# q8888620002/Group-Attribution-for-Diffusion-Models

Measured on AMD Instinct MI355X. Metric: shapley_coalitions_per_hour, higher is better.
Workload: dtype f32; 1 GPU; CIFAR-20 DDPM sFT coalition (BASELINE configs[1]): gd_steps=1000 @B=128 + 10240 samples x 100 DDIM steps @B=32 (32 batches fused/launch), UNet2DModel widths [128, 256, 256, 256] 35.75M params fp32; step = 1/1000 coalition = 1 train step + 1 sampler step @B=1024, enqueued on 3 HIP streams (the train step belongs to a later coalition: independent work); coalitions_in_flight=3

## Files before the change

### group-attribution-for-diffusion-models_amd/csrc/norm.hip

```cpp
#include "gad_reduce.h"
#include "gemm_dev.h"

namespace {

constexpr int NT = 256;
constexpr int MAXC = 3072;

struct Geo {
  int B, HW, C, G, cpg, C4, tpr, rows_par, nch, ppc;
};

static Geo make_geo(const gad_groupnorm_args* a) {
  Geo g;
  g.B = a->B; g.HW = a->HW; g.C = a->C; g.G = a->G;
  g.cpg = a->C / a->G;
  g.C4 = a->C / 4;
  g.tpr = g.C4 < NT ? g.C4 : NT;
  g.rows_par = NT / g.tpr;
  int nch = 2048 / (a->B > 0 ? a->B : 1);
  int maxch = a->HW / (8 * g.rows_par > 32 ? 8 * g.rows_par : 32);
  if (nch > maxch) nch = maxch;
  if (nch < 1) nch = 1;
  g.ppc = (a->HW + nch - 1) / nch;
  g.nch = (a->HW + g.ppc - 1) / g.ppc;
  return g;
}

__device__ __forceinline__ const float* gn_src(const float* x, const float* x2, int C1, int C, int HW, int b, int c0, int* stride) {
  if (x2 == nullptr || c0 < C1) {
    const int w = x2 ? C1 : C;
    *stride = w;
    return x + ((long)b * HW) * w + c0;
  }
  *stride = C - C1;
  return x2 + ((long)b * HW) * (C - C1) + (c0 - C1);
}

__device__ __forceinline__ bool gn_far_mean(const f32x4& mu, const f32x4& rs) {
  const f32x4 t = (mu * rs) * (mu * rs);
  return !(fmaxf(fmaxf(t[0], t[1]), fmaxf(t[2], t[3])) <= GN_COND - 1.f);
}
__global__ __launch_bounds__(NT) void gn_stats_kernel(const float* __restrict__ x, float* __restrict__ part, Geo g,
                                                      const float* __restrict__ x2, int C1) {
  __shared__ float red[2 * MAXC];
  __shared__ float s_mean[256];
  __shared__ int s_ill;
  if (threadIdx.x == 0) s_ill = 0;
  int b = blockIdx.x / g.nch, ch = blockIdx.x - b * g.nch;
  int p0 = ch * g.ppc, p1 = min(g.HW, p0 + g.ppc);
  int tid = threadIdx.x;
  int prow = tid / g.tpr, cfirst = tid - prow * g.tpr;
  if (prow < g.rows_par) {
// ... 399 lines not shown
  __syncthreads();
  f32x4* img4 = reinterpret_cast<f32x4*>(gn_img);
  if (act) {
    const float r1 = s_rstd[q / s.qpg], m2 = s_mean[q / s.qpg];
    const f32x4 rs = f32x4{r1, r1, r1, r1}, mu2 = f32x4{m2, m2, m2, m2};
    const f32x4 ga = *reinterpret_cast<const f32x4*>(gamma + c0), be = *reinterpret_cast<const f32x4*>(beta + c0);
    const f32x4 scale = ga * rs, shift = be - scale * mu2;
    const bool far = gn_far_mean(mu2, rs);
#pragma unroll
    for (int i = 0; i < NV; ++i) {
      int p = pl + i * s.PL;
      if (p < s.HW) {
        f32x4 z = far ? (v[i] - mu2) * scale + be : v[i] * scale + shift;
        if (silu) {
#pragma unroll
          for (int e = 0; e < 4; ++e) z[e] = silu_f(z[e]);
        }
        const int yy = p / w.W, xx = p - yy * w.W;
        img4[(yy * w.W + (xx ^ ((xx >> 2) & 1))) * s.qpr + q] = z;
      }
    }
  }
  __syncthreads();
  const int H = s.HW / w.W;
  const int items = w.TH * w.TW * s.qpr;
  for (int it = tid; it < items; it += NTH) {
    const int tile = it / s.qpr, qq = it - tile * s.qpr;
    const int ty = tile / w.TW, tx = tile - ty * w.TW;
    f32x4 t[6][6];
#pragma unroll
    for (int dx = 0; dx < 6; ++dx) {
      const int xx = 4 * tx - 1 + dx;
      const bool xok = xx >= 0 && xx < w.W;
      const int xs = xx ^ ((xx >> 2) & 1);
      f32x4 d[6], col[6];
#pragma unroll
      for (int dy = 0; dy < 6; ++dy) {
        const int yy = 4 * ty - 1 + dy;
        const bool ok = xok && yy >= 0 && yy < H;
        d[dy] = ok ? img4[(yy * w.W + xs) * s.qpr + qq] : f32x4{0.f, 0.f, 0.f, 0.f};
      }
      gadk::wino4_bt(d, col);
#pragma unroll
      for (int i = 0; i < 6; ++i) t[i][dx] = col[i];
    }
    float* out = w.V + ((long)b * (w.TH * w.TW) + tile) * s.C + sl * s.SC + qq * 4;
#pragma unroll
    for (int i = 0; i < 6; ++i) {
      f32x4 vv[6];
      gadk::wino4_bt(t[i], vv);
#pragma unroll
      for (int j = 0; j < 6; ++j) *reinterpret_cast<f32x4*>(out + (long)(6 * i + j) * w.pos_stride) = vv[j];
    }
  }
}

static int make_slab_wino(const gad_groupnorm_args* a, SlabGeo* out) {
  const int cpg = a->C / a->G, nth = 512;
  if (cpg % 4 != 0) return 0;
  int best_nv = 0;
  long best_score = -1;
  for (int k = 1; k * cpg <= a->C && k <= 64; ++k) {
    const int SC = k * cpg;
    if (a->C % SC != 0 || SC % 32 != 0) continue;
    if ((long)a->HW * SC * 4 > 128 * 1024) break;
    const int qpr = SC / 4;
    if (qpr > nth) break;
    const int PL = nth / qpr, nv = (a->HW + PL - 1) / PL;
    if (nv > 16) continue;
    const long blocks = (long)a->B * (a->C / SC);
    const long score = (blocks >= 512 ? (1L << 40) : blocks << 16) + SC;
    if (score > best_score) {
      best_score = score;
      best_nv = nv;
      int P2 = 1;
      while (P2 < PL) P2 <<= 1;
      *out = SlabGeo{a->HW, a->C, a->G, cpg, SC, qpr, PL, P2, a->C / SC, k, cpg / 4, 0};
    }
  }
  return !best_nv ? 0 : best_nv <= 4 ? 4 : best_nv <= 8 ? 8 : 16;
}

__device__ __forceinline__ float act_grad(float dy, float z, int silu) {
  if (!silu) return dy;
  float s = 1.f / (1.f + expf(-z));
  return dy * s * (1.f + z * (1.f - s));
}

template <int NV, int NTH>
__global__ __launch_bounds__(NTH) void gn_bwd_slab_kernel(const float* __restrict__ x, const float* __restrict__ dy,
                                                          float* __restrict__ dx, const float* __restrict__ gamma,
                                                          const float* __restrict__ beta, const float* __restrict__ mean,
                                                          const float* __restrict__ rstd, float* __restrict__ part,
                                                          SlabGeo s, int silu, const float* __restrict__ dx_add) {
  __shared__ f32x4 red_a[NTH], red_b[NTH];
  __shared__ float s_m1[64], s_m2[64];
  int b, sl;
  slab_of_block(s, b, sl);
  const int tid = threadIdx.x;
  const int pl = tid / s.qpr, q = tid - pl * s.qpr;
  const bool act = pl < s.PL;
  const int c0 = sl * s.SC + (act ? q : 0) * 4;
  const long base = ((long)b * s.HW) * s.C + c0;
  int gi[4];
  f32x4 mu, rs;
#pragma unroll
// ... 237 lines not shown
  dim3 grid(a->B * g.nch), block(NT);
  hipLaunchKernelGGL(gn_stats_kernel, grid, block, 0, st, a->x, (float*)a->ws, g, a->x2, a->C1);
  GAD_LAUNCH_CHECK("gn_stats");
  hipLaunchKernelGGL(gn_apply_kernel, grid, block, 0, st, a->x, a->y, a->gamma, a->beta, (const float*)a->ws, a->mean, a->rstd, g, a->eps, a->silu,
                     a->x2, a->C1);
  GAD_LAUNCH_CHECK("gn_apply");
  return 0;
}


static bool gn_wino_shapes_ok(const gad_groupnorm_args* a, int32_t W) {
  if (!a || a->B <= 0 || a->HW <= 0 || a->C <= 0 || a->G <= 0 || a->C % a->G != 0 || a->C % 32 != 0 || a->G > 256) return false;
  if (W <= 0 || a->HW % W != 0 || (W & 3) || ((a->HW / W) & 3)) return false;
  if (a->x2 && !(a->C1 > 0 && a->C1 < a->C && a->C1 % 4 == 0 && (a->C - a->C1) % 4 == 0)) return false;
  return true;
}
extern "C" int gad_groupnorm_wino4_ok(const gad_groupnorm_args* a, int32_t W) {
  SlabGeo sg;
  return gn_wino_shapes_ok(a, W) && make_slab_wino(a, &sg) ? 1 : 0;
}
extern "C" int gad_groupnorm_silu_wino4(const gad_groupnorm_args* a, float* V, int32_t W, void* stream) {
  GAD_CHECK(a && a->x && a->gamma && a->beta && a->mean && a->rstd && V, "gad_groupnorm_silu_wino4: null pointer");
  GAD_CHECK(gn_wino_shapes_ok(a, W), "gad_groupnorm_silu_wino4: shapes outside the plan (C %% 32, W and H multiples of 4; C=%d G=%d HW=%d W=%d)", a->C, a->G, a->HW, W);
  GAD_CHECK(gad_aligned16(a->x) && gad_aligned16(V) && gad_aligned16(a->gamma) && gad_aligned16(a->beta) && (!a->x2 || gad_aligned16(a->x2)),
            "gad_groupnorm_silu_wino4: pointers must be 16-byte aligned");
  SlabGeo sg;
  const int nv = make_slab_wino(a, &sg);
  GAD_CHECK(nv, "gad_groupnorm_silu_wino4: no slab plan (gad_groupnorm_wino4_ok tells)");
  GnWino w;
  w.V = V; w.W = W; w.TH = (a->HW / W) / 4; w.TW = W / 4;
  w.pos_stride = (long)a->B * w.TH * w.TW * a->C;
  const int c1 = a->x2 ? a->C1 : a->C;
  const int bytes = a->HW * sg.SC * (int)sizeof(float);
  hipStream_t st = (hipStream_t)stream;
  dim3 grid(a->B * sg.nslab), block(512);
#define GAD_GNW(NV_)                                                                                                        \
  do {                                                                                                                      \
    static int lds_set = 0;                                                                                                 \
    if (bytes > lds_set) {                                                                                                  \
      hipError_t e = hipFuncSetAttribute(reinterpret_cast<const void*>(gn_wino4_kernel<NV_>), hipFuncAttributeMaxDynamicSharedMemorySize, bytes); \
      GAD_CHECK(e == hipSuccess, "gad_groupnorm_silu_wino4: cannot reserve %d bytes of LDS: %s", bytes, hipGetErrorString(e)); \
      lds_set = bytes;                                                                                                      \
    }                                                                                                                       \
    hipLaunchKernelGGL((gn_wino4_kernel<NV_>), grid, block, bytes, st, a->x, a->x2, c1, a->gamma, a->beta, a->mean, a->rstd, sg, a->eps, a->silu, w); \
  } while (0)
  if (nv == 4) GAD_GNW(4);
  else if (nv == 8) GAD_GNW(8);
  else GAD_GNW(16);
#undef GAD_GNW
  GAD_LAUNCH_CHECK("gn_wino4");
  return 0;
}

extern "C" int gad_groupnorm_silu_bwd(const gad_groupnorm_args* a, void* stream) {
  if (check(a, "gad_groupnorm_silu_bwd")) return 1;
  GAD_CHECK(a->dy && gad_aligned16(a->dy) && ((a->dgamma == nullptr) == (a->dbeta == nullptr)), "gad_groupnorm_silu_bwd: null/unaligned grad pointer");
  GAD_CHECK(!a->dx_add || gad_aligned16(a->dx_add), "gad_groupnorm_silu_bwd: dx_add must be 16-byte aligned");
  Geo g = make_geo(a);
  hipStream_t st = (hipStream_t)stream;
  if (!(a->flags & GAD_GN_TWO_PASS)) {
    SlabGeo sg;
    int nth = NT, nv = make_slab(a, &sg, NT, 16);
    if (!nv) { nth = 512; nv = make_slab(a, &sg, 512, 16); }
    if (nv) {
      float* part = (float*)a->ws;
      dim3 sgrid(a->B * sg.nslab);
#define GAD_GNB(NV_, NTH_) hipLaunchKernelGGL((gn_bwd_slab_kernel<NV_, NTH_>), sgrid, dim3(NTH_), 0, st, a->x, a->dy, a->y, a->gamma, \
                                              a->beta, a->mean, a->rstd, part, sg, a->silu, a->dx_add)
      if (nth == NT) {
        if (nv <= 4) GAD_GNB(4, NT);
        else GAD_GNB(16, NT);
      } else {
        GAD_GNB(16, 512);
      }
#undef GAD_GNB
      GAD_LAUNCH_CHECK("gn_bwd_slab");
      if (a->dgamma) {
        float* ws2 = part + (long)a->B * a->C * 2;
        gad_reduce::launch(part, a->dbeta, a->dgamma, 1, (long)a->B, 2 * a->C, ws2, st);
        GAD_LAUNCH_CHECK("gn_bwd_param");
      }
      return 0;
    }
  }
  dim3 grid(a->B * g.nch), block(NT);
  hipLaunchKernelGGL(gn_bwd_stats_kernel, grid, block, 0, st, a->x, a->dy, a->gamma, a->beta, a->mean, a->rstd, (float*)a->ws, g, a->silu);
  GAD_LAUNCH_CHECK("gn_bwd_stats");
  hipLaunchKernelGGL(gn_bwd_apply_kernel, grid, block, 0, st, a->x, a->dy, a->y, a->gamma, a->beta, a->mean, a->rstd, (const float*)a->ws, g, a->silu, a->dx_add);
  GAD_LAUNCH_CHECK("gn_bwd_apply");
  if (a->dgamma) {
    float* ws2 = (float*)a->ws + (long)a->B * g.nch * a->C * 2;
    gad_reduce::launch((const float*)a->ws, a->dbeta, a->dgamma, 1, (long)a->B * g.nch, 2 * a->C, ws2, st);
    GAD_LAUNCH_CHECK("gn_bwd_param");
  }
  return 0;
}
```

### group-attribution-for-diffusion-models_amd/gad/_capi.py

```python
import ctypes as C
import os

_HERE = os.path.dirname(os.path.abspath(__file__))
LIB_PATH = os.path.join(_HERE, "libgad_hip.so")


class GadError(RuntimeError):
    pass


class ConvGeom(C.Structure):
    _fields_ = [("H", C.c_int32), ("W", C.c_int32), ("C", C.c_int32), ("ldx", C.c_int32),
                ("Ho", C.c_int32), ("Wo", C.c_int32), ("KH", C.c_int32), ("KW", C.c_int32),
                ("stride", C.c_int32), ("pad_t", C.c_int32), ("pad_l", C.c_int32), ("upsample", C.c_int32)]


class GemmArgs(C.Structure):
    _fields_ = [("A", C.c_void_p), ("B", C.c_void_p), ("C", C.c_void_p),
                ("a_mode", C.c_int32), ("b_mode", C.c_int32),
                ("M", C.c_int32), ("N", C.c_int32), ("K", C.c_int32),
                ("lda", C.c_int32), ("ldb", C.c_int32), ("ldc", C.c_int32),
                ("batch", C.c_int32), ("batch_inner", C.c_int32),
                ("strideA0", C.c_int64), ("strideA1", C.c_int64), ("strideB0", C.c_int64),
                ("strideB1", C.c_int64), ("strideC0", C.c_int64), ("strideC1", C.c_int64),
# ... 58 lines not shown

class JLArgs(C.Structure):
    _fields_ = [("A", C.c_void_p), ("lda", C.c_int64), ("G", C.c_int32), ("P", C.c_int64), ("p0", C.c_int64),
                ("d", C.c_int32), ("seed", C.c_uint32), ("model_id", C.c_uint32), ("type", C.c_int32),
                ("accumulate", C.c_int32), ("out", C.c_void_p), ("workspace", C.c_void_p), ("workspace_bytes", C.c_int64)]


class HGemmSegArgs(C.Structure):
    _fields_ = [("A", C.c_void_p), ("B", C.c_void_p), ("C", C.c_void_p), ("ws", C.c_void_p), ("ws_bytes", C.c_int64),
                ("c_seg_stride", C.c_int64), ("M", C.c_int32), ("N", C.c_int32), ("L", C.c_int32), ("S", C.c_int32),
                ("lda", C.c_int32), ("ldb", C.c_int32), ("ldc", C.c_int32), ("alpha", C.c_float), ("accumulate", C.c_int32),
                ("splitk_hint", C.c_int32)]


class LoraDropoutArgs(C.Structure):
    _fields_ = [("x", C.c_void_p), ("ldx", C.c_int64), ("M", C.c_int64), ("C", C.c_int32), ("r", C.c_int32),
                ("n_proj", C.c_int32), ("layer", C.c_uint32), ("A", C.c_void_p * 4), ("mid", C.c_void_p * 4),
                ("dmid", C.c_void_p * 4), ("dA", C.c_void_p * 4), ("dx", C.c_void_p), ("ld_dx", C.c_int64), ("p", C.c_double),
                ("scale", C.c_float), ("seed", C.c_uint32), ("offset", C.c_uint32), ("max_blocks", C.c_int32),
                ("workspace", C.c_void_p), ("workspace_bytes", C.c_int64)]


JL_NORMAL, JL_RADEMACHER = 0, 1
POOL_MAX, POOL_AVG, POOL_AVG_VALID = 0, 1, 2
GELU_ERF, GELU_QUICK = 0, 1
SIM_X_F32, SIM_X_U8 = 0, 1

GEMM_NO_PATCH, GEMM_TAP_MAJOR_K, GEMM_SCALAR_EPILOGUE, GEMM_GENERAL_LOADERS, GN_TWO_PASS = 1, 2, 4, 8, 1
GEMM_NO_WINO = 16
GEMM_WINO_WGRAD = 32
GEMM_WINO_ONLY_INPUT, GEMM_WINO_SKIP_INPUT = 64, 128
A_KC, A_MC, A_CONV, A_CONVT = 0, 1, 2, 3
B_KC, B_MC, B_WDGRAD, B_CONV = 0, 1, 2, 3

_vp, _i32, _i64, _f32, _f64 = C.c_void_p, C.c_int32, C.c_int64, C.c_float, C.c_double

SIGNATURES = {
    "gad_version": (C.c_int, []),
    "gad_last_error": (C.c_char_p, []),
    "gad_gemm_workspace_bytes": (_i64, [C.POINTER(GemmArgs)]),
    "gad_gemm": (C.c_int, [C.POINTER(GemmArgs), _vp]),
    "gad_gemm_uses_bf16": (C.c_int, [C.POINTER(GemmArgs)]),
    "gad_gemm_kernel_id": (C.c_int, [C.POINTER(GemmArgs)]),
    "gad_gemm_wino_bytes": (_i64, [C.POINTER(GemmArgs)]),
    "gad_wino_weights": (C.c_int, [_vp, _vp, _vp, _i64, _vp]),
    "gad_wino4_weights": (C.c_int, [_vp, _vp, _vp, _i64, _vp]),
    "gad_groupnorm_one_pass": (C.c_int, [C.POINTER(GroupNormArgs)]),
    "gad_gemm_plan": (C.c_int, [C.POINTER(GemmArgs), C.POINTER(_i32), C.POINTER(_i32), C.POINTER(_i32)]),
    "gad_groupnorm_workspace_bytes": (_i64, [C.POINTER(GroupNormArgs)]),
    "gad_groupnorm_silu_fwd": (C.c_int, [C.POINTER(GroupNormArgs), _vp]),
    "gad_groupnorm_silu_bwd": (C.c_int, [C.POINTER(GroupNormArgs), _vp]),
    "gad_groupnorm_wino4_ok": (C.c_int, [C.POINTER(GroupNormArgs), C.c_int32]),
    "gad_groupnorm_silu_wino4": (C.c_int, [C.POINTER(GroupNormArgs), _vp, C.c_int32, _vp]),
    "gad_attention_supported": (C.c_int, [_i32]),
    "gad_attention_uses_bf16": (C.c_int, [C.POINTER(AttentionArgs), _i32]),
    "gad_attention_bwd_workspace_bytes": (_i64, [C.POINTER(AttentionArgs)]),
    "gad_attention_fwd": (C.c_int, [C.POINTER(AttentionArgs), _vp]),
    "gad_attention_bwd": (C.c_int, [C.POINTER(AttentionArgs), _vp]),
    "gad_attention_d512_supported": (C.c_int, [_i32]),
    "gad_attention_fwd_d512": (C.c_int, [C.POINTER(AttentionArgs), _vp]),
    "gad_attention_causal_supported": (C.c_int, [_i32, _i32]),
    "gad_attention_causal_fwd": (C.c_int, [C.POINTER(AttentionArgs), _vp]),
    "gad_softmax_fwd": (C.c_int, [_vp, _vp, _i64, _i32, _f32, _vp]),
    "gad_softmax_bwd": (C.c_int, [_vp, _vp, _vp, _i64, _i32, _f32, _vp]),
    "gad_layernorm_workspace_bytes": (_i64, [_i64, _i32]),
    "gad_layernorm_fwd": (C.c_int, [_vp, _vp, _vp, _vp, _vp, _vp, _i64, _i32, _f32, _vp]),
    "gad_layernorm_bwd": (C.c_int, [_vp, _vp, _vp, _vp, _vp, _vp, _vp, _vp, _i64, _i32, _vp, _i64, _vp]),
    "gad_geglu_fwd": (C.c_int, [_vp, _vp, _i64, _i32, _vp]),
    "gad_geglu_bwd": (C.c_int, [_vp, _vp, _vp, _i64, _i32, _vp]),
    "gad_timestep_embedding": (C.c_int, [_vp, _vp, _i32, _i32, _i32, _f32, _f32, _vp]),
    "gad_rotate_conv3x3": (C.c_int, [_vp, _vp, _vp, _i32, _vp]),
    "gad_silu_fwd": (C.c_int, [_vp, _vp, _i64, _vp]),
    "gad_silu_bwd": (C.c_int, [_vp, _vp, _vp, _i64, _vp]),
    "gad_concat_channels": (C.c_int, [_vp, _vp, _vp, _i64, _i32, _i32, _vp]),
    "gad_split_channels": (C.c_int, [_vp, _vp, _vp, _i64, _i32, _i32, _vp]),
    "gad_nchw_to_nhwc": (C.c_int, [_vp, _vp, _i32, _i32, _i32, _vp]),
    "gad_nhwc_to_nchw": (C.c_int, [_vp, _vp, _i32, _i32, _i32, _vp]),
    "gad_upsample2x_bwd": (C.c_int, [_vp, _vp, _i32, _i32, _i32, _i32, _vp]),
    "gad_colsum": (C.c_int, [_vp, _vp, _i32, _i64, _i32, _vp, _i64, _vp]),
    "gad_add_noise": (C.c_int, [_vp, _vp, _vp, _vp, _vp, _i32, _i64, _vp]),
    "gad_ddim_step": (C.c_int, [_vp, _vp, _vp, _i64, _f32, _f32, _f32, _vp]),
    "gad_cfg_ddim_step": (C.c_int, [_vp, _vp, _vp, _i64, _f32, _f32, _f32, _f32, _vp]),
    "gad_to_image01": (C.c_int, [_vp, _vp, _i64, _vp]),
    "gad_mse_fwd_bwd": (C.c_int, [_vp, _vp, _vp, _vp, _i64, _f32, _vp, _i64, _vp]),
    "gad_sumsq": (C.c_int, [_vp, _vp, _i64, _vp, _i64, _vp]),
    "gad_clip_adam_ema": (C.c_int, [C.POINTER(AdamArgs), _vp]),
    "gad_ema_update": (C.c_int, [_vp, _vp, _i64, _f32, _vp]),
    "gad_hgemm_workspace_bytes": (_i64, [C.POINTER(HGemmArgs)]),
    "gad_hgemm_plan": (C.c_int, [C.POINTER(HGemmArgs), C.POINTER(_i32), C.POINTER(_i32)]),
    "gad_hgemm": (C.c_int, [C.POINTER(HGemmArgs), _vp]),
    "gad_hgemm_tn_workspace_bytes": (_i64, [C.POINTER(HGemmArgs)]),
    "gad_hgemm_tn": (C.c_int, [C.POINTER(HGemmArgs), _vp]),
    "gad_hgemm_tn_seg_workspace_bytes": (_i64, [C.POINTER(HGemmSegArgs)]),
    "gad_hgemm_tn_seg": (C.c_int, [C.POINTER(HGemmSegArgs), _vp]),
    "gad_h_transpose": (C.c_int, [_vp, _vp, _i32, _i32, _i32, _i32, _i32, _vp]),
    "gad_h_cast": (C.c_int, [_vp, _vp, _i64, _i32, _vp]),
    "gad_h_shadow_pairs": (C.c_int, [_vp, _vp, _vp, _vp, _i32, _vp]),
    "gad_h_add": (C.c_int, [_vp, _vp, _vp, _i64, _vp]),
    "gad_h_groupnorm_workspace_bytes": (_i64, [C.POINTER(GroupNormArgs)]),
    "gad_h_groupnorm_silu_fwd": (C.c_int, [C.POINTER(GroupNormArgs), _vp]),
    "gad_h_groupnorm_silu_bwd": (C.c_int, [C.POINTER(GroupNormArgs), _vp]),
    "gad_h_layernorm_fwd": (C.c_int, [_vp, _vp, _vp, _vp, _vp, _vp, _i64, _i32, _f32, _vp]),
    "gad_h_layernorm_bwd": (C.c_int, [_vp, _vp, _vp, _vp, _vp, _vp, _vp, _i64, _i32, _vp]),
    "gad_h_geglu_fwd": (C.c_int, [_vp, _vp, _i64, _i32, _vp]),
    "gad_h_geglu_bwd": (C.c_int, [_vp, _vp, _vp, _i64, _i32, _vp]),
    "gad_h_upsample2x_bwd": (C.c_int, [_vp, _vp, _i32, _i32, _i32, _i32, _vp]),
# ... 58 lines not shown
```

### group-attribution-for-diffusion-models_amd/gad/ops.py

```python
from __future__ import annotations

import ctypes as C
import math
from typing import Optional

import torch

from . import _capi
from ._capi import (A_CONV, A_CONVT, A_KC, A_MC, B_CONV, B_KC, B_MC, B_WDGRAD, AdamArgs, ConvGeom, GemmArgs,
                    GroupNormArgs, check)
from .shadows import (WEIGHT_EPOCH, Shadow, cached, in_flat_buffer as _in_flat_buffer, weight_key, written,
                      written_everywhere)

_WS = {}
WS_BYTES = 1 << 30


def _stream():
    return C.c_void_p(torch.cuda.current_stream().cuda_stream)


_raw_stream = getattr(torch._C, "_cuda_getCurrentRawStream", None)


# ... 49 lines not shown

def _sink(param):
    if _PER_SAMPLE[0] is not None and param is not None and param.requires_grad:
        raise _capi.GadError("per-sample gradient sink: only the LoRA matrices of the half-precision activation path have "
                             "per-sample gradients (csrc/half.hip: gad_hgemm_tn_seg)")
    v = getattr(param, "_gad_sink", None) if (param is not None and _SINK_ACTIVE[0]) else None
    if v is None:
        return None, True
    first = getattr(param, "_gad_sink_epoch", -1) != _SINK_EPOCH[0]
    param._gad_sink_epoch = _SINK_EPOCH[0]
    return v, first


def _deliver(param, grad):
    v, first = _sink(param)
    if v is None:
        return grad
    if first:
        v.copy_(grad)
    else:
        v.add_(grad)
    return None


OPERAND_PRECISION = [0]


class operand_precision:

    def __init__(self, name):
        if name not in ("f32", "fp32", "no", "bf16", "bf16-operands", "bf16-activations"):
            raise ValueError(f"operand precision {name!r}: use 'f32', 'bf16' (= 'bf16-activations') or 'bf16-operands'")
        self.value = {"bf16": 2, "bf16-activations": 2, "bf16-operands": 1}.get(name, 0)

    def __enter__(self):
        self.prev = OPERAND_PRECISION[0]
        OPERAND_PRECISION[0] = self.value
        return self

    def __exit__(self, *exc):
        OPERAND_PRECISION[0] = self.prev
        return False


def set_operand_precision(name):
    OPERAND_PRECISION[0] = 0 if name in (None, "no", "f32", "fp32") else operand_precision("bf16" if name in ("fp16", "bf16") else name).value


def half_activations() -> bool:
    return OPERAND_PRECISION[0] == 2


KERNEL_FLAGS = {"gemm": 0, "gn": 0, "native_dgrad": False, "two_kernel_attn_bwd": False, "narrow_attn_fwd": False, "no_wino4": False,
                "no_gn_wino": False}


class kernel_flags:

    def __init__(self, no_patch=False, tap_major_k=False, gn_two_pass=False, scalar_epilogue=False, general_loaders=False,
                 native_dgrad=False, two_kernel_attn_bwd=False, narrow_attn_fwd=False, no_wino=False, no_wino4=False, no_gn_wino=False):
        gemm = ((_capi.GEMM_NO_PATCH if no_patch else 0) | (_capi.GEMM_TAP_MAJOR_K if tap_major_k else 0)
                | (_capi.GEMM_NO_WINO if no_wino else 0)
                | (_capi.GEMM_SCALAR_EPILOGUE if scalar_epilogue else 0)
                | (_capi.GEMM_GENERAL_LOADERS if general_loaders else 0))
        self.values = {"gemm": gemm, "gn": _capi.GN_TWO_PASS if gn_two_pass else 0, "native_dgrad": native_dgrad,
                       "two_kernel_attn_bwd": two_kernel_attn_bwd, "narrow_attn_fwd": narrow_attn_fwd, "no_wino4": no_wino4,
                       "no_gn_wino": no_gn_wino}

    def __enter__(self):
        self.prev = dict(KERNEL_FLAGS)
        KERNEL_FLAGS.update(self.values)
        return self

    def __exit__(self, *exc):
        KERNEL_FLAGS.update(self.prev)
        return False


SCRATCH_ALLOC = None
OUT_ALLOC = None
OUT_ALLOC_DT = None


ROUTE_STATS = None


def _scratch(kind, nbytes, device):
    if SCRATCH_ALLOC is not None:
        return SCRATCH_ALLOC(kind, nbytes, device)
    return torch.empty(nbytes, dtype=torch.uint8, device=device)


def _out(shape, device):
    if OUT_ALLOC is not None:
        return OUT_ALLOC(tuple(shape), device)
    return torch.empty(tuple(shape), device=device, dtype=torch.float32)


def gemm_raw(A, B, Cout, a_mode, b_mode, M, N, K, lda, ldb, ldc, *, geom: Optional[ConvGeom] = None, alpha=1.0,
             bias=None, rowadd=None, rows_per_group=1, residual=None, ldr=0, batch=1, batch_inner=1,
             sA=(0, 0), sB=(0, 0), sC=(0, 0), tile_hint=0, splitk_hint=0, A2=None, a_split=0, B_bf16=None,
             A_k2=None, B_k2=None, k_split=0, force_f32=False, launch=True) -> GemmArgs:
    ws = workspace(A.device)
    a = GemmArgs()
    a.A, a.B, a.C = A.data_ptr(), B.data_ptr(), Cout.data_ptr()
    a.a_mode, a.b_mode = a_mode, b_mode
    a.M, a.N, a.K = M, N, K
    a.lda, a.ldb, a.ldc = lda, ldb, ldc
    a.batch, a.batch_inner = batch, batch_inner
    a.strideA0, a.strideA1 = sA
    a.strideB0, a.strideB1 = sB
    a.strideC0, a.strideC1 = sC
    if geom is not None:
        a.g = geom
    a.alpha = alpha
    a.bias, a.rowadd, a.residual = _ptr(bias), _ptr(rowadd), _ptr(residual)
    a.rows_per_group = rows_per_group
    a.ld_rowadd = (rowadd.stride(0) if rowadd.ndim == 2 else rowadd.shape[-1]) if rowadd is not None else 0
    a.ldr = ldr
    a.ws, a.ws_bytes = ws.data_ptr(), ws.numel()
# ... 255 lines not shown

def _offer_wino(a, device, w, form, supplied=False):
    U = wino_weight(w, form, offered=True) if form else None
    if U is None:
        return None
    setattr(a, "B_wino" if form == 2 else "B_wino4", U.data_ptr())
    need = _capi.load().gad_gemm_wino_bytes(C.byref(a))
    if not need or (supplied and form != 4):
        a.B_wino = a.B_wino4 = None
        return None
    V = _scratch("wino", need, device)
    a.wino_ws, a.wino_ws_bytes = V.data_ptr(), need
    if form == 4:
        a.flags |= _capi.GEMM_WINO_SKIP_INPUT if supplied else 0
        _count_wino4(a, 6)
    return V


def _opt_in_wino_wgrad(a, device, wino_v):
    a.flags |= _capi.GEMM_WINO_WGRAD
    need = _capi.load().gad_gemm_wino_bytes(C.byref(a))
    if not need:
        a.flags &= ~_capi.GEMM_WINO_WGRAD
        return None
    ws = _scratch("wino", need, device)
    a.wino_ws, a.wino_ws_bytes = ws.data_ptr(), need
    if wino_v is not None and wino_v.numel() >= 36 * (a.K // 16) * a.g.C * 4:
        a.B_wino4 = wino_v.data_ptr()
        a.flags |= _capi.GEMM_WINO_SKIP_INPUT
    _count_wino4(a, 7)
    return ws


def gn_silu_conv3x3_raw(x, x2, gamma, beta, G, eps, w, bias, rowadd=None, residual=None, tile_hint=0):
    _req(x, "groupnorm x")
    Bn, H, W, C1 = x.shape
    Cin = C1 + (x2.shape[-1] if x2 is not None else 0)
    lib = _capi.load()

    def plain():
        h = group_norm_cat_raw(x, x2, gamma, beta, G, eps, True) if x2 is not None else group_norm(x, gamma, beta, G, eps, True)
        return conv2d_fwd_raw(h, w, bias, 1, (1, 1, 1, 1), False, rowadd=rowadd, residual=residual, tile_hint=tile_hint)
    form = wino_prefilter(w.shape[2:], 1, (1, 1, 1, 1), False, w.shape[0], Cin, (H, W), tile_hint)[0]
    if torch.is_grad_enabled() or w.shape[1] != Cin or KERNEL_FLAGS["gn"] or KERNEL_FLAGS["no_gn_wino"] or H % 4 or W % 4 or not form:
        return plain()
    mean = torch.empty((Bn, G), device=x.device, dtype=torch.float32)
    rstd = torch.empty_like(mean)
    gn = GroupNormArgs()
    gn.x, gn.gamma, gn.beta, gn.mean, gn.rstd = x.data_ptr(), gamma.data_ptr(), beta.data_ptr(), mean.data_ptr(), rstd.data_ptr()
    gn.B, gn.HW, gn.C, gn.G, gn.eps, gn.silu = Bn, H * W, Cin, G, eps, 1
    if x2 is not None:
        _req(x2, "groupnorm x2")
        gn.x2, gn.C1 = x2.data_ptr(), C1
    if not lib.gad_groupnorm_wino4_ok(C.byref(gn), W):
        return plain()
    y, a = _conv_fwd_args(x, (Bn, H, W, Cin), w, bias, 1, (1, 1, 1, 1), False, rowadd, residual, tile_hint, 0)
    V = _offer_wino(a, x.device, w, form, supplied=True)
    if V is None:
        return plain()
    check(lib.gad_groupnorm_silu_wino4(C.byref(gn), V.data_ptr(), W, _stream()), "gad_groupnorm_silu_wino4")
    _launch_gemm(a, x.device)
    return y


def _wino_shadow(src, items, f):
    launch, npos = (_capi.load().gad_wino_weights, 16) if f == 2 else (_capi.load().gad_wino4_weights, 36)
    rows, where, doff = [], {}, 0
    for off, co, ci in items:
        where[off] = (doff, npos * co * ci)
        rows += [(off, doff, co, ci, a, b) for a in range(0, co, 32) for b in range(0, ci, 32)]
        doff += npos * co * ci
    U = torch.empty(max(doff, 1), device=src.device, dtype=torch.float32)
    table = torch.tensor(rows, dtype=torch.int64, device=src.device)
    return Shadow((U,), lambda home: check(launch(home.data_ptr(), U.data_ptr(), table.data_ptr(), len(rows), _stream()),
                                           "gad_wino_weights"), where)


def wino_weight(w, f=2, offered=False):
    co, ci = w.shape[0], w.shape[1]
    if not offered and wino_prefilter(w.shape[2:], 1, (1, 1, 1, 1), False, co, ci, (f, f))[0] != f:
        return None
    attr = "_gad_wino" if f == 2 else "_gad_wino4"
    if _in_flat_buffer(w):
        flat, off, n = w._gad_flat
        s = getattr(flat, attr, None)
        if s is None:
            s = _wino_shadow(flat, [it for it in _conv3x3_residents(flat) if _wino_ok(it[1], it[2])], f)
            setattr(flat, attr, s)
        if off not in s.where:
            return None
        d0, dn = s.where[off]
        return s.fresh_for(flat, off, w).buffers[0][d0:d0 + dn]
    return cached(w, attr, lambda: _wino_shadow(w, [(0, co, ci)], f), lambda s: s.refresh(weight_krsc(w))).buffers[0]


def refresh_wino(module):
    for p in module.parameters():
        if p.ndim == 4 and tuple(p.shape[2:]) == (3, 3):
            home = p._gad_flat[0] if _in_flat_buffer(p) else p
            for f, attr in ((2, "_gad_wino"), (4, "_gad_wino4")):
                if getattr(home, attr, None) is not None:
                    wino_weight(p, f)


def _dense_1x1(KH, KW, stride, pad, upsample, Cin, Cout) -> bool:
    return (KH == 1 and KW == 1 and stride == 1 and tuple(pad) == (0, 0, 0, 0) and not upsample and Cin % 4 == 0 and Cout % 4 == 0
            and not KERNEL_FLAGS["gemm"] & _capi.GEMM_GENERAL_LOADERS)


def two_source_ok(c1: int, c2: int) -> bool:
    return c1 % 32 == 0 and c2 % 32 == 0


# ... 1190 lines not shown
```

### include/gad.h

```cpp
#ifndef GAD_H
#define GAD_H
#include <stdint.h>
#ifdef __cplusplus
extern "C" {
#endif

int gad_version(void);
const char* gad_last_error(void);

enum gad_a_mode {
  GAD_A_KC = 0,
  GAD_A_MC = 1,
  GAD_A_CONV = 2,
  GAD_A_CONVT = 3
};
enum gad_b_mode {
  GAD_B_KC = 0,
  GAD_B_MC = 1,
  GAD_B_WDGRAD = 2,
  GAD_B_CONV = 3
};

typedef struct gad_conv_geom {
  int32_t H, W, C;
// ... 36 lines not shown
  const float* B_wino;
  void* wino_ws;
  int64_t wino_ws_bytes;
  const float* B_wino4;
} gad_gemm_args;
enum gad_gemm_flags {
  GAD_GEMM_NO_WINO = 16,
  GAD_GEMM_WINO_WGRAD = 32,
  GAD_GEMM_NO_PATCH = 1,
  GAD_GEMM_TAP_MAJOR_K = 2,
  GAD_GEMM_SCALAR_EPILOGUE = 4,
  GAD_GEMM_GENERAL_LOADERS = 8,
  GAD_GEMM_WINO_ONLY_INPUT = 64,
  GAD_GEMM_WINO_SKIP_INPUT = 128
};

int64_t gad_gemm_workspace_bytes(const gad_gemm_args* a);
int gad_gemm_plan(const gad_gemm_args* a, int32_t* tile, int32_t* splitk, int32_t* vec);
int gad_gemm(const gad_gemm_args* a, void* stream);
int gad_gemm_uses_bf16(const gad_gemm_args* a);
int gad_gemm_kernel_id(const gad_gemm_args* a);
int64_t gad_gemm_wino_bytes(const gad_gemm_args* a);
int gad_wino_weights(const float* src, float* dst, const int64_t* table, int64_t n_tiles, void* stream);
int gad_wino4_weights(const float* src, float* dst, const int64_t* table, int64_t n_tiles, void* stream);

typedef struct gad_groupnorm_args {
  const float* x;
  float* y;
  const float* gamma;
  const float* beta;
  float* mean;
  float* rstd;
  const float* dy;
  float* dgamma;
  float* dbeta;
  int32_t B, HW, C, G;
  float eps;
  int32_t silu;
  void* ws;
  int64_t ws_bytes;
  const float* x2;
  int32_t C1;
  int32_t flags;
  const float* dx_add;
} gad_groupnorm_args;
enum gad_groupnorm_flags { GAD_GN_TWO_PASS = 1 };

int64_t gad_groupnorm_workspace_bytes(const gad_groupnorm_args* a);
int gad_groupnorm_one_pass(const gad_groupnorm_args* a);
int gad_groupnorm_silu_fwd(const gad_groupnorm_args* a, void* stream);
int gad_groupnorm_silu_bwd(const gad_groupnorm_args* a, void* stream);
int gad_groupnorm_wino4_ok(const gad_groupnorm_args* a, int32_t W);
int gad_groupnorm_silu_wino4(const gad_groupnorm_args* a, float* V, int32_t W, void* stream);

typedef struct gad_attention_args {
  const float* q; const float* k; const float* v;
  float* o;
  float* lse;
  const float* d_o;
  float* delta;
  float* dq; float* dk; float* dv;
  int32_t B, heads, Tq, Tk, d;
  int32_t ldq, ldk, ldv, ldo, ld_do, ld_dq, ld_dk, ld_dv;
  int64_t stride_q, stride_k, stride_v, stride_o, stride_do, stride_dq, stride_dk, stride_dv;
  float scale;
  int32_t operand_precision;
  void* ws;
  int64_t ws_bytes;
  int32_t flags;
} gad_attention_args;
#define GAD_ATTN_TWO_KERNEL_BWD 1
#define GAD_ATTN_NARROW_FWD 2
int64_t gad_attention_bwd_workspace_bytes(const gad_attention_args* a);
int gad_attention_supported(int32_t d);
int gad_attention_uses_bf16(const gad_attention_args* a, int32_t backward);
int gad_attention_fwd(const gad_attention_args* a, void* stream);
int gad_attention_bwd(const gad_attention_args* a, void* stream);
int gad_attention_d512_supported(int32_t d);
int gad_attention_fwd_d512(const gad_attention_args* a, void* stream);
int gad_attention_causal_supported(int32_t T, int32_t d);
int gad_attention_causal_fwd(const gad_attention_args* a, void* stream);

int gad_softmax_fwd(const float* s, float* p, int64_t rows, int32_t n, float scale, void* stream);
int gad_softmax_bwd(const float* p, const float* dp, float* ds, int64_t rows, int32_t n, float scale,
                    void* stream);

int64_t gad_layernorm_workspace_bytes(int64_t rows, int32_t C);
int gad_layernorm_fwd(const float* x, float* y, const float* gamma, const float* beta, float* mean, float* rstd,
                      int64_t rows, int32_t C, float eps, void* stream);
int gad_layernorm_bwd(const float* x, const float* dy, float* dx, const float* dx_add, const float* gamma, const float* mean,
                      const float* rstd, float* dgamma_dbeta, int64_t rows, int32_t C, void* ws, int64_t ws_bytes,
                      void* stream);
int gad_geglu_fwd(const float* h, float* out, int64_t M, int32_t F, void* stream);
int gad_geglu_bwd(const float* h, const float* dout, float* dh, int64_t M, int32_t F, void* stream);

int gad_timestep_embedding(const int64_t* t, float* out, int32_t B, int32_t dim, int32_t flip_sin_to_cos,
                           float freq_shift, float max_period, void* stream);
int gad_silu_fwd(const float* x, float* y, int64_t n, void* stream);
int gad_silu_bwd(const float* x, const float* dy, float* dx, int64_t n, void* stream);
int gad_rotate_conv3x3(const float* src, float* dst, const int64_t* table, int32_t n_tiles, void* stream);
int gad_concat_channels(const float* a, const float* b, float* out, int64_t pixels, int32_t C1, int32_t C2,
                        void* stream);
int gad_split_channels(const float* d, float* da, float* db, int64_t pixels, int32_t C1, int32_t C2,
                       void* stream);
int gad_nchw_to_nhwc(const float* x, float* y, int32_t B, int32_t C, int32_t HW, void* stream);
int gad_nhwc_to_nchw(const float* x, float* y, int32_t B, int32_t C, int32_t HW, void* stream);
// ... 193 lines not shown
```

Before: 44.46 coalitions/hour.

## Add banded GroupNorm+SiLU Winograd input transform for shapes the slab path rejects

Adds a fallback path for GroupNorm+SiLU fused into the Winograd F(4,3) input transform. It computes stats in a separate kernel plus a finish kernel, then a banded kernel loads 32-channel slabs into LDS, normalises them and writes the transformed tiles. It is used when the existing whole-slab fused kernel rejects the shape (large images or LDS limits), which previously fell back to separate GroupNorm and conv. The cost is two extra small launches and some halo rows loaded twice across bands.

```diff
diff --git a/group-attribution-for-diffusion-models_amd/csrc/norm.hip b/group-attribution-for-diffusion-models_amd/csrc/norm.hip
--- a/group-attribution-for-diffusion-models_amd/csrc/norm.hip
+++ b/group-attribution-for-diffusion-models_amd/csrc/norm.hip
@@ -1,3 +1,5 @@
+#include <type_traits>
+
 #include "gad_reduce.h"
 #include "gemm_dev.h"
 
@@ -503,6 +505,106 @@
 #pragma unroll
       for (int j = 0; j < 6; ++j) *reinterpret_cast<f32x4*>(out + (long)(6 * i + j) * w.pos_stride) = vv[j];
     }
+  }
+}
+
+__global__ __launch_bounds__(NT) void gn_finish_kernel(const float* __restrict__ part, float* __restrict__ mean_out,
+                                                       float* __restrict__ rstd_out, Geo g, float eps) {
+  __shared__ float s_mean[256], s_rstd[256];
+  const int b = blockIdx.x;
+  gn_combine(part, g, b, eps, s_mean, s_rstd);
+  __syncthreads();
+  for (int grp = threadIdx.x; grp < g.G; grp += NT) {
+    mean_out[b * g.G + grp] = s_mean[grp];
+    rstd_out[b * g.G + grp] = s_rstd[grp];
+  }
+}
+
+constexpr int GNL_SC = 32, GNL_Q = GNL_SC / 4;
+__global__ __launch_bounds__(256) void gn_wino4_load_kernel(const float* __restrict__ x, const float* __restrict__ x2, int C1,
+                                                            const float* __restrict__ gamma, const float* __restrict__ beta,
+                                                            const float* __restrict__ mean, const float* __restrict__ rstd,
+                                                            Geo g, int silu, GnWino w, int TB) {
+  extern __shared__ __attribute__((aligned(16))) float gnl_img[];
+  f32x4* img4 = reinterpret_cast<f32x4*>(gnl_img);
+  const int nslab = g.C / GNL_SC, nband = (w.TH + TB - 1) / TB;
+  int bid = blockIdx.x;
+  const int sl = bid % nslab;
+  bid /= nslab;
+  const int band = bid % nband, b = bid / nband;
+  const int tid = threadIdx.x, q = tid & (GNL_Q - 1);
+  const int c0 = sl * GNL_SC + q * 4;
+  const int H = g.HW / w.W;
+  const int ty0 = band * TB, tb = min(TB, w.TH - ty0);
+  const int y0 = 4 * ty0 - 1, rows = 4 * tb + 2;
+  const f32x4 ga = *reinterpret_cast<const f32x4*>(gamma + c0), be = *reinterpret_cast<const f32x4*>(beta + c0);
+  f32x4 mu, rs;
+#pragma unroll
+  for (int e = 0; e < 4; ++e) {
+    const int grp = (c0 + e) / g.cpg;
+    mu[e] = mean[b * g.G + grp];
+    rs[e] = rstd[b * g.G + grp];
+  }
+  const f32x4 scale = rs * ga, shift = be - mu * scale;
+  const bool far = gn_far_mean(mu, rs);
+  int ldx;
+  const float* xb = gn_src(x, x2, C1, g.C, g.HW, b, c0, &ldx);
+  const int npx = rows * w.W;
+  constexpr int NLD = 10;
+  for (int base = tid / GNL_Q; base < npx; base += NLD * (256 / GNL_Q)) {
+    f32x4 v[NLD];
+#pragma unroll
+    for (int u = 0; u < NLD; ++u) {
+      const int px = min(base + u * (256 / GNL_Q), npx - 1);
+      const int row = px / w.W, xx = px - row * w.W;
+      v[u] = *reinterpret_cast<const f32x4*>(xb + (long)(min(max(y0 + row, 0), H - 1) * w.W + xx) * ldx);
+    }
+#pragma unroll
+    for (int u = 0; u < NLD; ++u) {
+      const int px = base + u * (256 / GNL_Q);
+      const int row = px / w.W, xx = px - row * w.W;
+      const int yy = y0 + row;
+      f32x4 z = far ? (v[u] - mu) * scale + be : v[u] * scale + shift;
+      if (silu) {
+#pragma unroll
+        for (int e = 0; e < 4; ++e) z[e] = silu_f(z[e]);
+      }
+      if (px < npx) img4[(row * w.W + (xx ^ ((xx >> 2) & 1))) * GNL_Q + q] = (yy >= 0 && yy < H) ? z : f32x4{0.f, 0.f, 0.f, 0.f};
+    }
+  }
+  __syncthreads();
+  const int items = tb * w.TW * GNL_Q;
+  auto half_rows = [&](auto half_c, int it) {
+    constexpr int I0 = 3 * decltype(half_c)::value;
+    const int qq = it & (GNL_Q - 1), tile = it / GNL_Q;
+    const int tyl = tile / w.TW, tx = tile - tyl * w.TW;
+    f32x4 t[3][6];
+#pragma unroll
+    for (int dx = 0; dx < 6; ++dx) {
+      const int xx = 4 * tx - 1 + dx;
+      const bool xok = xx >= 0 && xx < w.W;
+      const int xc = xok ? xx : 0;
+      const int xs = xc ^ ((xc >> 2) & 1);
+      f32x4 d[6], col[6];
+#pragma unroll
+      for (int dy = 0; dy < 6; ++dy)
+        d[dy] = xok ? img4[((4 * tyl + dy) * w.W + xs) * GNL_Q + qq] : f32x4{0.f, 0.f, 0.f, 0.f};
+      gadk::wino4_bt(d, col);
+#pragma unroll
+      for (int i = 0; i < 3; ++i) t[i][dx] = col[I0 + i];
+    }
+    float* out = w.V + (((long)b * w.TH + ty0 + tyl) * w.TW + tx) * g.C + sl * GNL_SC + qq * 4;
+#pragma unroll
+    for (int i = 0; i < 3; ++i) {
+      f32x4 vv[6];
+      gadk::wino4_bt(t[i], vv);
+#pragma unroll
+      for (int j = 0; j < 6; ++j) *reinterpret_cast<f32x4*>(out + (long)(6 * (I0 + i) + j) * w.pos_stride) = vv[j];
+    }
+  };
+  for (int u = tid; u < 2 * items; u += 256) {
+    if (u < items) half_rows(std::integral_constant<int, 0>{}, u);
+    else half_rows(std::integral_constant<int, 1>{}, u - items);
   }
 }
 
@@ -846,6 +948,42 @@
   return 0;
 }
 
+static int gn_load_band(int32_t W) {
+  for (int tb = 2; tb >= 1; --tb)
+    if ((long)(4 * tb + 2) * W * GNL_SC * 4 <= 64 * 1024) return tb;
+  return 0;
+}
+extern "C" int gad_groupnorm_wino4_load_ok(const gad_groupnorm_args* a, int32_t W) {
+  return gn_wino_shapes_ok(a, W) && a->C <= MAXC && (a->C / a->G) % 4 == 0 && gn_load_band(W) ? 1 : 0;
+}
+extern "C" int gad_groupnorm_silu_wino4_load(const gad_groupnorm_args* a, float* V, int32_t W, void* stream) {
+  GAD_CHECK(a && a->x && a->gamma && a->beta && a->mean && a->rstd && V, "gad_groupnorm_silu_wino4_load: null pointer");
+  GAD_CHECK(gad_groupnorm_wino4_load_ok(a, W),
+            "gad_groupnorm_silu_wino4_load: shapes outside the plan (C %% 32, C <= 3072, channels per group %% 4, W and H multiples of 4, W <= 84; C=%d G=%d HW=%d W=%d)",
+            a->C, a->G, a->HW, W);
+  GAD_CHECK(gad_aligned16(a->x) && gad_aligned16(V) && gad_aligned16(a->gamma) && gad_aligned16(a->beta) && (!a->x2 || gad_aligned16(a->x2)),
+            "gad_groupnorm_silu_wino4_load: pointers must be 16-byte aligned");
+  const int64_t need = gad_groupnorm_workspace_bytes(a);
+  GAD_CHECK(a->ws && a->ws_bytes >= need, "gad_groupnorm_silu_wino4_load: workspace too small (%lld < %lld)", (long long)a->ws_bytes, (long long)need);
+  hipStream_t st = (hipStream_t)stream;
+  const Geo g = make_geo(a);
+  hipLaunchKernelGGL(gn_stats_kernel, dim3(a->B * g.nch), dim3(NT), 0, st, a->x, (float*)a->ws, g, a->x2, a->C1);
+  GAD_LAUNCH_CHECK("gn_stats");
+  hipLaunchKernelGGL(gn_finish_kernel, dim3(a->B), dim3(NT), 0, st, (const float*)a->ws, a->mean, a->rstd, g, a->eps);
+  GAD_LAUNCH_CHECK("gn_finish");
+  GnWino w;
+  w.V = V; w.W = W; w.TH = (a->HW / W) / 4; w.TW = W / 4;
+  w.pos_stride = (long)a->B * w.TH * w.TW * a->C;
+  const int tb = gn_load_band(W);
+  const long blocks = (long)a->B * ((w.TH + tb - 1) / tb) * (a->C / GNL_SC);
+  GAD_CHECK(blocks < (1L << 31), "gad_groupnorm_silu_wino4_load: transform grid too large");
+  const int bytes = (4 * tb + 2) * W * GNL_SC * (int)sizeof(float);
+  hipLaunchKernelGGL(gn_wino4_load_kernel, dim3((unsigned)blocks), dim3(256), bytes, st, a->x, a->x2, a->C1,
+                     a->gamma, a->beta, (const float*)a->mean, (const float*)a->rstd, g, a->silu, w, tb);
+  GAD_LAUNCH_CHECK("gn_wino4_load");
+  return 0;
+}
+
 extern "C" int gad_groupnorm_silu_bwd(const gad_groupnorm_args* a, void* stream) {
   if (check(a, "gad_groupnorm_silu_bwd")) return 1;
   GAD_CHECK(a->dy && gad_aligned16(a->dy) && ((a->dgamma == nullptr) == (a->dbeta == nullptr)), "gad_groupnorm_silu_bwd: null/unaligned grad pointer");
diff --git a/group-attribution-for-diffusion-models_amd/gad/_capi.py b/group-attribution-for-diffusion-models_amd/gad/_capi.py
--- a/group-attribution-for-diffusion-models_amd/gad/_capi.py
+++ b/group-attribution-for-diffusion-models_amd/gad/_capi.py
@@ -134,6 +134,8 @@
     "gad_groupnorm_silu_bwd": (C.c_int, [C.POINTER(GroupNormArgs), _vp]),
     "gad_groupnorm_wino4_ok": (C.c_int, [C.POINTER(GroupNormArgs), C.c_int32]),
     "gad_groupnorm_silu_wino4": (C.c_int, [C.POINTER(GroupNormArgs), _vp, C.c_int32, _vp]),
+    "gad_groupnorm_wino4_load_ok": (C.c_int, [C.POINTER(GroupNormArgs), C.c_int32]),
+    "gad_groupnorm_silu_wino4_load": (C.c_int, [C.POINTER(GroupNormArgs), _vp, C.c_int32, _vp]),
     "gad_attention_supported": (C.c_int, [_i32]),
     "gad_attention_uses_bf16": (C.c_int, [C.POINTER(AttentionArgs), _i32]),
     "gad_attention_bwd_workspace_bytes": (_i64, [C.POINTER(AttentionArgs)]),
diff --git a/group-attribution-for-diffusion-models_amd/gad/ops.py b/group-attribution-for-diffusion-models_amd/gad/ops.py
--- a/group-attribution-for-diffusion-models_amd/gad/ops.py
+++ b/group-attribution-for-diffusion-models_amd/gad/ops.py
@@ -125,20 +125,21 @@
 
 
 KERNEL_FLAGS = {"gemm": 0, "gn": 0, "native_dgrad": False, "two_kernel_attn_bwd": False, "narrow_attn_fwd": False, "no_wino4": False,
-                "no_gn_wino": False}
+                "no_gn_wino": False, "no_gn_load": False, "gn_load": False}
 
 
 class kernel_flags:
 
     def __init__(self, no_patch=False, tap_major_k=False, gn_two_pass=False, scalar_epilogue=False, general_loaders=False,
-                 native_dgrad=False, two_kernel_attn_bwd=False, narrow_attn_fwd=False, no_wino=False, no_wino4=False, no_gn_wino=False):
+                 native_dgrad=False, two_kernel_attn_bwd=False, narrow_attn_fwd=False, no_wino=False, no_wino4=False, no_gn_wino=False,
+                 no_gn_load=False, gn_load=False):
         gemm = ((_capi.GEMM_NO_PATCH if no_patch else 0) | (_capi.GEMM_TAP_MAJOR_K if tap_major_k else 0)
                 | (_capi.GEMM_NO_WINO if no_wino else 0)
                 | (_capi.GEMM_SCALAR_EPILOGUE if scalar_epilogue else 0)
                 | (_capi.GEMM_GENERAL_LOADERS if general_loaders else 0))
         self.values = {"gemm": gemm, "gn": _capi.GN_TWO_PASS if gn_two_pass else 0, "native_dgrad": native_dgrad,
                        "two_kernel_attn_bwd": two_kernel_attn_bwd, "narrow_attn_fwd": narrow_attn_fwd, "no_wino4": no_wino4,
-                       "no_gn_wino": no_gn_wino}
+                       "no_gn_wino": no_gn_wino, "no_gn_load": no_gn_load, "gn_load": gn_load}
 
     def __enter__(self):
         self.prev = dict(KERNEL_FLAGS)
@@ -500,13 +501,19 @@
     if x2 is not None:
         _req(x2, "groupnorm x2")
         gn.x2, gn.C1 = x2.data_ptr(), C1
-    if not lib.gad_groupnorm_wino4_ok(C.byref(gn), W):
+    slab = bool(lib.gad_groupnorm_wino4_ok(C.byref(gn), W)) and not KERNEL_FLAGS["gn_load"]
+    if not slab and (KERNEL_FLAGS["no_gn_load"] or not lib.gad_groupnorm_wino4_load_ok(C.byref(gn), W)):
         return plain()
     y, a = _conv_fwd_args(x, (Bn, H, W, Cin), w, bias, 1, (1, 1, 1, 1), False, rowadd, residual, tile_hint, 0)
     V = _offer_wino(a, x.device, w, form, supplied=True)
     if V is None:
         return plain()
-    check(lib.gad_groupnorm_silu_wino4(C.byref(gn), V.data_ptr(), W, _stream()), "gad_groupnorm_silu_wino4")
+    if slab:
+        check(lib.gad_groupnorm_silu_wino4(C.byref(gn), V.data_ptr(), W, _stream()), "gad_groupnorm_silu_wino4")
+    else:
+        ws = workspace(x.device)
+        gn.ws, gn.ws_bytes = ws.data_ptr(), ws.numel()
+        check(lib.gad_groupnorm_silu_wino4_load(C.byref(gn), V.data_ptr(), W, _stream()), "gad_groupnorm_silu_wino4_load")
     _launch_gemm(a, x.device)
     return y
 
diff --git a/include/gad.h b/include/gad.h
--- a/include/gad.h
+++ b/include/gad.h
@@ -112,6 +112,8 @@
 int gad_groupnorm_silu_bwd(const gad_groupnorm_args* a, void* stream);
 int gad_groupnorm_wino4_ok(const gad_groupnorm_args* a, int32_t W);
 int gad_groupnorm_silu_wino4(const gad_groupnorm_args* a, float* V, int32_t W, void* stream);
+int gad_groupnorm_wino4_load_ok(const gad_groupnorm_args* a, int32_t W);
+int gad_groupnorm_silu_wino4_load(const gad_groupnorm_args* a, float* V, int32_t W, void* stream);
 
 typedef struct gad_attention_args {
   const float* q; const float* k; const float* v;
```

Result: no change. 44.61 coalitions/hour (median of 6 runs) (+0.3%).
